# pxl-th/Trace.jl

Measured on AMD Instinct MI355X. Metric: Mray/s (all bounces), higher is better.
Workload: dtype f32

## Files before the change

### trace.jl_amd/csrc/th_device.h

```cpp
#pragma once
#include "th_scene.h"

namespace th {

template <class T>
TH_D T uniform_load(const T* p, uint32_t i) {
#if defined(__HIP_DEVICE_COMPILE__)
    typedef const __attribute__((address_space(4))) T* ConstPtr;
    return ((ConstPtr)(uintptr_t)p)[i];
#else
    return p[i];
#endif
}


struct TriTest {
    float t;
    f3 bary;
};
TH_D bool tri_degenerate(f3 v0, f3 v1, f3 v2) {
    const f3 v = cross(v2 - v0, v1 - v0);
    return dot(v, v) == 0.0f;
}
struct RayShear {
// ... 438 lines not shown
        const float d_o = dot(wo, wh), d_i = dot(wi, wh);
        if (d_o * d_i > 0.0f) return 0.0f;
        const float denom = d_o + eta * d_i;
        const float dwh_dwi = fabs_(d_i * (eta * eta) / (denom * denom));
        return tr_pdf(l.a, l.b, wo, wh) * dwh_dwi;
    }
    default: return same_hemisphere(wo, wi) ? fabs_(cos_theta(wi)) * kInvPi : 0.0f;
    }
}
struct LobeSample {
    f3 wi;
    float pdf;
    f3 f;
    int sampled_type;
};
TH_D LobeSample lobe_sample_f(const Lobe& l, f3 wo, f2 u) {
    LobeSample s;
    s.wi = splat3(0.0f);
    s.pdf = 0.0f;
    s.f = splat3(0.0f);
    s.sampled_type = -1;
    switch (l.kind) {
    case LOBE_SPECULAR_R: {
        s.wi = mk3(-wo.x, -wo.y, wo.z);
        s.pdf = 1.0f;
        s.f = lobe_fresnel(l, cos_theta(s.wi)) * lobe_r(l) / fabs_(cos_theta(s.wi));
        return s;
    }
    case LOBE_SPECULAR_T: {
        const bool entering = cos_theta(wo) > 0.0f;
        const float eta_i = entering ? l.eta_a : l.eta_b;
        const float eta_t = entering ? l.eta_b : l.eta_a;
        f3 wi;
        if (!refract(wo, face_forward(mk3(0.0f, 0.0f, 1.0f), wo), eta_i / eta_t, wi)) return s;
        s.wi = wi;
        s.pdf = 1.0f;
        const float cos_wi = cos_theta(wi);
// ... 244 lines not shown
    if (wo.z == 0.0f) return r;
    f3 wi = cosine_sample_hemisphere(ur);
    if (wo.z < 0.0f) wi = mk3(wi.x, wi.y, -wi.z);
    const float pdf = same_hemisphere(wo, wi) ? fabs_(cos_theta(wi)) * kInvPi : 0.0f;
    if (pdf == 0.0f) return r;
    const f3 wi_w = bsdf_to_world(s, wi);
    const bool refl = (dot(wi_w, s.ng) * dot(wo_w, s.ng)) > 0.0f;
    f3 f = splat3(0.0f);
    if (refl) f = f + lobe_r(l) * kInvPi;
    r.wi = wi_w;
    r.f = f;
    r.pdf = pdf;
    r.sampled_type = l.type;
    return r;
}

struct LightSample {
    f3 radiance;
    f3 wi;
    float pdf;
};
template <bool DIRL>
TH_D LightSample sample_li(const LightRec& l, f3 p) {
    LightSample s;
    const f3 lp = mk3(l.position[0], l.position[1], l.position[2]);
    if (DIRL && l.kind == 2) {
        s.wi = lp;
        s.pdf = 1.0f;
        s.radiance = mk3(l.I[0], l.I[1], l.I[2]);
        return s;
// ... 33 lines not shown
```

### trace.jl_amd/csrc/th_host.h

```cpp
#pragma once
#include <hip/hip_runtime.h>

#include <algorithm>
#include <chrono>
#include <cstdarg>
#include <cstdio>
#include <cstdlib>
#include <cstring>
#include <memory>
#include <string>
#include <thread>
#include <type_traits>
#include <vector>

#include "th_options.h"
#include "th_owned.h"
#include "th_bvh.h"
#include "th_kernels.h"
#include "th_trace2.h"
#include "th_trace8.h"
#ifdef TRHIP_EXPERIMENTS
#include "th_trace4.h"
#include "th_trace7.h"
#endif
// ... 68 lines not shown
struct SceneGeometry {
    uint64_t id = 0;
    int max_node_primitives = -1;
    std::vector<MaterialRec> materials;
    std::vector<float> base_colour;
    std::vector<HostPrim> prims;
    std::vector<float> prim_tan, prim_uv;
    std::vector<SphereRec> spheres;
    std::vector<HostAABB> sphere_bounds;
    FlatBVH bvh;
    FlatBVH acc;
    std::vector<uint32_t> occ_slots;
    std::vector<float> occ_boxes;
    DevBuf d_leaf_boxes;
    DevBuf d_nodes, d_prims, d_nrm, d_tan, d_shade, d_spheres, d_materials, d_base_colour, d_wnodes, d_w8nodes, d_w8tris;
    DevBuf d_acc_w4nodes;
    DevBuf d_acc_wnodes, d_acc_prims, d_slot_boxes, d_sphere_boxes, d_sphere_slots, d_sphere_cert;
};
static_assert(!std::is_copy_constructible_v<SceneGeometry>, "SceneGeometry owns its device buffers");

struct SceneViews {
    bool has_materialless_prim = false;
    DeviceScene dev{};
    WideScene wide{};
    Wide8Scene w8{};
    uint32_t w8_nodes = 0, w8_depth = 0;
    bool partial_spheres = false;
    bool wide_ok = false;
    bool w8_ok = false;
    bool literal_only = false;
// ... 287 lines not shown
```

### trace.jl_amd/csrc/th_kernels.h

```cpp
#pragma once
#include "th_device.h"

namespace th {

constexpr int kBlock = 256;
constexpr int kStackLds = 32;
constexpr int kStackSpill = 32;

struct PathQueue {
    float4* o;
    float4* d;
    float4* beta;
};
struct ShadowQueue {
    float4* o;
    float4* d;
    float4* c;
};
constexpr int kMaxDepth = 62;
constexpr int kSeg = 32;
constexpr uint32_t kSegGran = 256;
#ifndef TH_CTR_STRIDE
#define TH_CTR_STRIDE 32
#endif
// ... 399 lines not shown
            occluded[i] = occ ? 1 : 0;
        }
    }
    if (ctr) {
        if (blockIdx.x == 0 && threadIdx.x == 0) atomicAdd(&ctr->shadow_total, (unsigned long long)seg_total(sv));
        if (COUNT) {
            const unsigned long long sn = wave_sum(nn), spr = wave_sum(np);
            if (lane_id() == 0) {
                atomicAdd(&ctr->nodes_shadow, sn);
                atomicAdd(&ctr->prims_shadow, spr);
            }
        }
    }
}

template <bool TRI_ONLY = false, bool TAN = true>
TH_D bool rebuild_shading(const DeviceScene& sc, int prim, f3 o, f3 d, Shading& sh, uint32_t& material, const float4* bary = nullptr, f3* fast_r = nullptr) {
    const float4* rec = sc.shade + 8 * (size_t)prim;
    const float4 p0 = rec[0], p1 = rec[1], p2 = rec[2];
    const float4 na = rec[3], nb = rec[4], nc = rec[5];
    const float4 cn = rec[6], cs = rec[7];
    const uint32_t meta = __float_as_uint(p0.w);
    material = meta & PRIM_MATERIAL_MASK;
    if (fast_r) *fast_r = mk3(na.w, nb.w, nc.w);
    if (!TRI_ONLY && (meta & PRIM_SPHERE)) {
        const SphereRec& s = sc.spheres[__float_as_uint(p0.x)];
        SphereHit h;
        if (!sphere_intersect<true>(s, o, d, kInf, h)) return false;
        sh = shade_sphere(s, h, d);
        return true;
    }
    const f3 v0 = mk3(p0.x, p0.y, p0.z), v1 = mk3(p1.x, p1.y, p1.z), v2 = mk3(p2.x, p2.y, p2.z);
    TriTest tt;
    if (bary)
        tt.bary = mk3(bary->z, bary->w, bary->x);
    else if (!tri_intersect<true>(v0, v1, v2, o, d, kInf, &tt))
        return false;
    const bool has_n = (meta & PRIM_HAS_NORMALS) != 0;
    const TriConstants tc{mk3(cn.x, cn.y, cn.z), mk3(cs.x, cs.y, cs.z)};
    const float4* tan = (TAN && sc.tri_tan && (meta & PRIM_HAS_TANGENTS)) ? sc.tri_tan + 3 * (size_t)prim : nullptr;
    sh = shade_triangle(v0, v1, v2, has_n, mk3(na.x, na.y, na.z), mk3(nb.x, nb.y, nb.z), mk3(nc.x, nc.y, nc.z), (meta & PRIM_FLIP) != 0, tt.bary, d, &tc, tan);
    return true;
}
template <int TH_ONE_COPY = 0> __global__ __launch_bounds__(kBlock) void k_shade_constants(float4* __restrict__ shade, const float4* __restrict__ prims, const float4* __restrict__ nrm, const float4* __restrict__ uv, uint32_t n_prims) {
    for (uint32_t k = blockIdx.x * kBlock + threadIdx.x; k < n_prims; k += gridDim.x * kBlock) {
        float4* rec = shade + 8 * (size_t)k;
        const float4 p0 = prims[3 * (size_t)k], p1 = prims[3 * (size_t)k + 1], p2 = prims[3 * (size_t)k + 2];
        rec[0] = p0;
        rec[1] = p1;
        rec[2] = p2;
        for (int j = 0; j < 3; ++j) rec[3 + j] = nrm[3 * (size_t)k + j];
        float4 c6 = make_float4(0.0f, 0.0f, 0.0f, 0.0f), c7 = c6;
        if (!(__float_as_uint(p0.w) & PRIM_SPHERE)) {
            float uvs[6];
            bool has_uv = false;
// ... 2 lines not shown
                uvs[0] = a.x, uvs[1] = a.y, uvs[2] = a.z, uvs[3] = a.w, uvs[4] = b.x, uvs[5] = b.y;
                has_uv = b.z != 0.0f;
            }
            const TriConstants tc = triangle_constants(mk3(p0.x, p0.y, p0.z), mk3(p1.x, p1.y, p1.z), mk3(p2.x, p2.y, p2.z), has_uv ? uvs : nullptr);
            c6 = make_float4(tc.n.x, tc.n.y, tc.n.z, 0.0f);
            c7 = make_float4(tc.ss.x, tc.ss.y, tc.ss.z, 0.0f);
        }
        rec[6] = c6;
        rec[7] = c7;
    }
}

#ifndef TH_SHADE_WAVES
#define TH_SHADE_WAVES 4
#endif
struct ShadeStream {
    const uint32_t* tags_in;
    uint32_t* tags_out;
    uint32_t term_stride;
    uint8_t* poison;
};
struct ShadeOut {
    bool want_shadow, want_next;
    float4 so4, sd4, sc4, no4, nd4, nb4;
    uint32_t next_depth;
};
template <bool STREAM, bool FAST, bool TAN = true, bool DIRL = false>
TH_D void shade_vertex(const DeviceScene& sc, const PathQueue& qin, const float4* __restrict__ hits, float4* __restrict__ L, uint32_t i, int depth_fixed, int max_depth,
                       uint32_t hits_have_bary, const ShadeStream& ss, ShadeOut& out) {
    const float4 h4 = hits[i];
    const int prim = __float_as_int(h4.y);
    const float4 o4 = qin.o[i], d4 = qin.d[i], b4 = qin.beta[i];
    const int depth = STREAM ? (int)ss.tags_in[i] : depth_fixed;
    const uint32_t slot = STREAM ? (uint32_t)(depth - 1) * ss.term_stride + __float_as_uint(o4.w) : __float_as_uint(o4.w);
    const f3 o = mk3(o4.x, o4.y, o4.z), d = mk3(d4.x, d4.y, d4.z);
    f3 beta = mk3(b4.x, b4.y, b4.z);
    Shading sh;
    uint32_t material;
    f3 fast_r;
    if (!(rebuild_shading<FAST, TAN>(sc, prim, o, d, sh, material, hits_have_bary ? &h4 : nullptr, &fast_r) && material != PRIM_NO_MATERIAL)) return;
    const LobeSet& bsdf = sc.materials[FAST ? 0u : material].set[1];
    const bool lambert = FAST || bsdf_is_single_lambert(bsdf);
    Lobe lam;
    if (FAST) {
        lam.kind = LOBE_LAMBERT_R;
        lam.type = BSDF_DIFFUSE | BSDF_REFLECTION;
        lam.r[0] = fast_r.x;
        lam.r[1] = fast_r.y;
        lam.r[2] = fast_r.z;
    } else if (lambert) {
        lam = bsdf.lobe[0];
    }
    const uint64_t key = ((uint64_t)__float_as_uint(b4.w) << 32) | (uint64_t)__float_as_uint(d4.w);
    const uint32_t v = (uint32_t)(depth - 1);
    const f3 wo = -d;
    const uint32_t poison = ((isnan_(beta.x) || isinf_(beta.x)) ? 1u : 0u) | ((isnan_(beta.y) || isinf_(beta.y)) ? 2u : 0u) | ((isnan_(beta.z) || isinf_(beta.z)) ? 4u : 0u);
    bool direct_added = false;
    if (sc.n_lights > 0) {
        const int nl = (int)sc.n_lights;
        int ln = (int)__builtin_ceilf(ts_uniform(key, ts_vertex_dim(v, TS_V_LIGHT_PICK)) * (float)nl);
        if (ln > nl) ln = nl;
        if (ln < 1) ln = 1;
        const float light_pdf = 1.0f / (float)nl;
        const LightRec light = nl == 1 ? uniform_load(sc.lights, 0u) : sc.lights[ln - 1];
        const LightSample ls = sample_li<DIRL>(light, sh.p);
        if (ls.pdf > 0.0f && !is_black(ls.radiance)) {
            const f3 f = (lambert ? lambert_bsdf_f(lam, sh, sh.wo, ls.wi) : bsdf_f(bsdf, sh, sh.wo, ls.wi, BSDF_ALL & ~BSDF_SPECULAR)) * fabs_(dot(ls.wi, sh.ns));
            if (!is_black(f)) {
                const f3 fl = f * ls.radiance;
                const f3 Ld1 = splat3(0.0f) + (ls.pdf == 1.0f ? fl : fl / ls.pdf);
                const f3 Ld = light_pdf == 1.0f ? Ld1 : Ld1 / light_pdf;
                const f3 c = beta * Ld;
                const f3 lp = light_target<DIRL>(light, sh.p);
// ... 8 lines not shown
            }
        }
    }
    if (!direct_added && poison && ss.poison) {
        ss.poison[slot] |= (uint8_t)poison;
    } else if (!direct_added && poison) {
        float4 l = L[slot];
        const float nanv = __builtin_nanf("");
        if (poison & 1u) l.x += nanv;
        if (poison & 2u) l.y += nanv;
        if (poison & 4u) l.z += nanv;
        L[slot] = l;
    }
    if (depth < max_depth) {
        const f2 u{ts_uniform(key, ts_vertex_dim(v, TS_V_BSDF_U0)), ts_uniform(key, ts_vertex_dim(v, TS_V_BSDF_U1))};
        const BsdfSample bs = lambert ? lambert_bsdf_sample_f(lam, sh, wo, u) : bsdf_sample_f(bsdf, sh, wo, u, BSDF_ALL);
        if (!(bs.pdf == 0.0f || is_black(bs.f))) {
            beta = beta * (bs.f * fabs_(dot(bs.wi, sh.ns)) / bs.pdf);
            const float by = to_Y(beta);
            bool alive = true;
            if (by < 0.25f) {
                const float cont = jmin(1.0f, by);
                if (ts_uniform(key, ts_vertex_dim(v, TS_V_RR)) > cont)
                    alive = false;
                else
                    beta = beta / cont;
            }
            if (alive) {
                const f3 org = sh.p + 1e-6f * bs.wi;
                const f3 nd = check_direction(bs.wi);
                out.no4 = make_float4(org.x, org.y, org.z, o4.w);
                out.nd4 = make_float4(nd.x, nd.y, nd.z, d4.w);
                out.nb4 = make_float4(beta.x, beta.y, beta.z, b4.w);
                out.next_depth = (uint32_t)(depth + 1);
                out.want_next = true;
            }
        }
    }
}

template <bool STREAM, bool TAN = true, bool DIRL = false>
__global__ __launch_bounds__(kBlock) __attribute__((amdgpu_waves_per_eu(TH_SHADE_WAVES))) void k_shade_path(DeviceScene sc, const DeviceSensor* __restrict__ sep, PathQueue qin, PathQueue qout, ShadowQueue sq, uint32_t cap,
                                                       const float4* __restrict__ hits, float4* __restrict__ L, Counters* ctr, int row, int depth_fixed, int max_depth, uint32_t hits_have_bary,
                                                       ShadeStream ss) {
    __shared__ SegView sv;
    __shared__ uint32_t s_ring[kBlock / 64][128];
    const SegQueue qv{ctr->n_queue[row], cap, 0u};
    seg_load(qv, sv);
    const uint32_t total = sv.prefix[kSeg];
    const uint32_t lane = lane_id(), wv = threadIdx.x >> 6;
    const unsigned long long lt_mask = (1ull << lane) - 1ull;
    const uint32_t seg_out = ((blockIdx.x * kBlock + threadIdx.x) >> 6) % kSeg;
    uint32_t ring_head = 0, ring_cnt = 0;
    auto emit = [&](const ShadeOut& e) {
        uint32_t si, ni;
        wave_compact2(e.want_shadow, &ctr->n_shadow[row][seg_out * kCtrStride], e.want_next, &ctr->n_queue[row + 1][seg_out * kCtrStride], si, ni);
        si += seg_out * cap;
        ni += seg_out * cap;
        if (e.want_shadow) {
            sq.o[si] = e.so4;
            sq.d[si] = e.sd4;
            sq.c[si] = e.sc4;
        }
        if (e.want_next) {
            qout.o[ni] = e.no4;
            qout.d[ni] = e.nd4;
            qout.beta[ni] = e.nb4;
            if (STREAM) ss.tags_out[ni] = e.next_depth;
        }
    };
    uint32_t seg_in = 0;
    for (uint32_t flat = blockIdx.x * kBlock + threadIdx.x; flat < total; flat += gridDim.x * kBlock) {
        uint32_t lb;
        seg_locate_from(sv, flat & ~63u, seg_in, lb);
        const uint32_t local = lb + (flat & 63u);
        const uint32_t i = seg_in * cap + local;
        int cls = 0;
        if (local < sv.count[seg_in]) {
            const int prim = __float_as_int(hits[i].y);
            if (prim >= 0) {
                cls = (__float_as_uint(sc.shade[8 * (size_t)prim].w) & PRIM_FAST) ? 1 : 2;
            }
        }
        ShadeOut e;
        e.want_shadow = e.want_next = false;
        e.next_depth = 0;
        if (cls == 1) shade_vertex<STREAM, true, TAN, DIRL>(sc, qin, hits, L, i, depth_fixed, max_depth, hits_have_bary, ss, e);
        emit(e);
        const unsigned long long m2 = __ballot(cls == 2);
        if (m2) {
            if (cls == 2) s_ring[wv][(ring_head + ring_cnt + (uint32_t)__popcll(m2 & lt_mask)) & 127u] = i;
            ring_cnt += (uint32_t)__popcll(m2);
            __builtin_amdgcn_fence(__ATOMIC_ACQ_REL, "wavefront");
            if (ring_cnt >= 64u) {
                const uint32_t j = s_ring[wv][(ring_head + lane) & 127u];
                ShadeOut g;
                g.want_shadow = g.want_next = false;
                g.next_depth = 0;
                shade_vertex<STREAM, false, TAN, DIRL>(sc, qin, hits, L, j, depth_fixed, max_depth, hits_have_bary, ss, g);
                emit(g);
                ring_head = (ring_head + 64u) & 127u;
                ring_cnt -= 64u;
                __builtin_amdgcn_fence(__ATOMIC_ACQ_REL, "wavefront");
            }
        }
    }
    if (ring_cnt) {
        ShadeOut g;
        g.want_shadow = g.want_next = false;
        g.next_depth = 0;
        if (lane < ring_cnt) shade_vertex<STREAM, false, TAN, DIRL>(sc, qin, hits, L, s_ring[wv][(ring_head + lane) & 127u], depth_fixed, max_depth, hits_have_bary, ss, g);
        emit(g);
    }
}
template <int TH_ONE_COPY = 0> __global__ __launch_bounds__(kBlock) void k_fold_terms(const float4* __restrict__ terms, uint64_t n_slots, uint32_t n_depths, float4* __restrict__ L) {
    for (uint64_t i = (uint64_t)blockIdx.x * kBlock + threadIdx.x; i < n_slots; i += (uint64_t)gridDim.x * kBlock) {
        float4 l = make_float4(0.0f, 0.0f, 0.0f, 0.0f);
        for (uint32_t dd = 0; dd < n_depths; ++dd) {
            const float4 t = terms[(uint64_t)dd * n_slots + i];
            l.x += t.x;
            l.y += t.y;
            l.z += t.z;
        }
        L[i] = l;
    }
}
template <int TH_ONE_COPY = 0> __global__ __launch_bounds__(kBlock) void k_fill_u32(uint32_t* __restrict__ p, uint64_t n, uint32_t v) {
// ... 503 lines not shown
```

### trace.jl_amd/csrc/th_scene.h

```cpp
#pragma once
#include "th_math.h"

namespace th {

enum : uint32_t {
    PRIM_SPHERE = 1u << 24,
    PRIM_HAS_NORMALS = 1u << 25,
    PRIM_FLIP = 1u << 26,
    PRIM_DEGENERATE = 1u << 27,
    PRIM_FAST = 1u << 28,
    PRIM_HAS_TANGENTS = 1u << 29,
    PRIM_MATERIAL_MASK = 0x00ffffffu,
    PRIM_NO_MATERIAL = 0x00ffffffu
};

struct SphereRec {
    float o2w[16];
    float o2w_inv[16];
    float radius, z_min, z_max, theta_min, theta_max, phi_max;
    uint32_t flip;
    uint32_t never_clipped;
};

enum LobeKind : int32_t { LOBE_LAMBERT_R = 0, LOBE_OREN_NAYAR = 1, LOBE_SPECULAR_R = 2, LOBE_SPECULAR_T = 3, LOBE_FRESNEL_SPECULAR = 4, LOBE_MICROFACET_R = 5, LOBE_MICROFACET_T = 6, LOBE_LAMBERT_T = 7 };
enum : int32_t { BSDF_NONE = 0, BSDF_REFLECTION = 1, BSDF_TRANSMISSION = 2, BSDF_DIFFUSE = 4, BSDF_GLOSSY = 8, BSDF_SPECULAR = 16, BSDF_ALL = 31 };
enum : int32_t { FRESNEL_NOOP = 0, FRESNEL_DIELECTRIC = 1 };
// ... 27 lines not shown
};
static_assert(sizeof(LightRec) == 112, "LightRec: the single-light path loads it through scalar loads (th_kernels.h)");

struct DeviceScene {
    const float4* nodes;
    const float4* prims;
    const float4* tri_nrm;
    const float4* tri_tan;
    const float4* shade;
    const SphereRec* spheres;
    const MaterialRec* materials;
    const LightRec* lights;
    uint32_t n_nodes, n_prims, n_spheres, n_materials, n_lights;
};

struct DeviceSensor {
    float raster_to_camera[16];
    float camera_to_world[16];
    float lens_radius, focal_distance, shutter_open, shutter_close;
    float crop_min[2], crop_max[2];
    float filter_radius[2];
    float scale;
    int32_t sb_min[2], sb_max[2];
    int32_t sb_w, sb_h;
    int32_t film_w, film_h;
    int32_t tiles_x, tiles_y;
    int32_t band_y0, band_rows, band_ty0, band_ty1, accumulate;
};

}
// ... 1 lines not shown
```

### trace.jl_amd/csrc/tu_path.hip

```cpp
#include "th_host.h"
#include "th_adaptive.h"

void derive_sensor(const trhip_sensor* sn, DeviceSensor& d) {
    std::memcpy(d.raster_to_camera, sn->raster_to_camera, sizeof d.raster_to_camera);
    std::memcpy(d.camera_to_world, sn->camera_to_world, sizeof d.camera_to_world);
    d.lens_radius = sn->lens_radius;
    d.focal_distance = sn->focal_distance;
    d.shutter_open = sn->shutter_open;
    d.shutter_close = sn->shutter_close;
    for (int i = 0; i < 2; ++i) {
        d.crop_min[i] = sn->crop_min[i];
        d.crop_max[i] = sn->crop_max[i];
        d.filter_radius[i] = sn->filter_radius[i];
        d.sb_min[i] = (int)std::floor(sn->crop_min[i] + 0.5f - sn->filter_radius[i]);
        d.sb_max[i] = (int)std::ceil(sn->crop_max[i] - 0.5f + sn->filter_radius[i]);
    }
    d.scale = sn->scale;
    d.sb_w = d.sb_max[0] - d.sb_min[0] + 1;
    d.sb_h = d.sb_max[1] - d.sb_min[1] + 1;
    d.film_w = (int)std::fabs(sn->crop_max[0] - (sn->crop_min[0] - 1.0f));
    d.film_h = (int)std::fabs(sn->crop_max[1] - (sn->crop_min[1] - 1.0f));
    d.tiles_x = (int)std::floor(((float)(d.sb_max[0] - d.sb_min[0]) + 16.0f) / 16.0f);
    d.tiles_y = (int)std::floor(((float)(d.sb_max[1] - d.sb_min[1]) + 16.0f) / 16.0f);
    d.band_y0 = d.sb_min[1];
    d.band_rows = d.sb_h;
    d.band_ty0 = 0;
    d.band_ty1 = d.tiles_y - 1;
    d.accumulate = 0;
}

bool film_packed(const DeviceSensor& ds) { return std::fmax(ds.filter_radius[0], ds.filter_radius[1]) <= 1.0f && ds.filter_radius[0] > 0.0f && ds.filter_radius[1] > 0.0f; }
static double film_sample_bytes(bool packed) { return packed ? 16.0 : 24.0; }
int ensure_film_samples(trhip_ctx* ctx, bool packed, uint64_t total_slots) { return packed ? 0 : ensure(ctx, ctx->pfilm, total_slots * sizeof(float2)); }
static uint64_t film_padded_slots(const DeviceSensor& ds, uint32_t spp) { return (((uint64_t)ds.sb_w * ds.band_rows + 63u) / 64u) * 64u * spp; }
static bool film_fusable(const DeviceSensor& ds, uint32_t spp) { return film_packed(ds) && film_padded_slots(ds, spp) < (1ull << 32); }
static bool film_fused(const trhip_ctx* ctx, const DeviceSensor& ds, uint32_t spp) { return ctx->opt.film_fused && ctx->opt.film_relayout && film_fusable(ds, spp); }
static FilmSideTable film_side_table(trhip_ctx* ctx, hipStream_t st, uint64_t total_slots, bool* ok) {
    const uint32_t side_cap = (uint32_t)std::min<uint64_t>(total_slots / 16 + 65536, 0x7ffffff0ull);
    *ok = ensure(ctx, ctx->film_side, ((size_t)side_cap + 1) * sizeof(uint4)) == 0;
    if (!*ok) return FilmSideTable{nullptr, nullptr, 0};
    (void)hipMemsetAsync(ctx->film_side.p, 0, sizeof(uint4), st);
    return FilmSideTable{(uint4*)ctx->film_side.p + 1, (uint32_t*)ctx->film_side.p, side_cap};
}
void launch_film(trhip_ctx* ctx, hipStream_t st, const DeviceSensor& ds, const DeviceSensor* dsp, const float4* L, uint64_t total_slots, uint32_t spp, uint64_t seed, uint32_t sample_offset,
                 float4* d_film, bool fused, const MapFrame* map) {
// ... 192 lines not shown
        HIP_TRY(ctx, hipMemcpyAsync(frozen, ctr->n_queue[r], row_bytes, hipMemcpyDeviceToDevice, ps));
        HIP_TRY(ctx, hipMemsetAsync(&lc[out_pg], 0, sizeof(uint32_t), ps));
        HIP_TRY(ctx, hipMemsetAsync(&lc[2], 0, sizeof(uint32_t), ps));
        StreamCtl sc_c{list_of(0, in_pg), list_of(0, out_pg), &lc[in_pg], &lc[2], &lc[out_pg], budget_min, ctx->opt.stream_budget_shift, pq[cur].beta, tags[cur], pq[cur].o, pq[cur].d, pq[cur].beta, hits, tags[cur],
                       ctr->n_queue[r], cap};
        const SegQueue qc{frozen, cap, 0u};
        const TraceOut oc{hits, nullptr, nullptr, nullptr, 1u};
        tm.begin(1, ps);
        launch_trace2_stream(ctx, ps, scene, false, qc, pq[cur].o, pq[cur].d, oc, ctr->work_closest[r], pp.overflow[0].p, ctr, sc_c);
        tm.end(1, ps);
        if (ps2 != ps && r > 0) HIP_TRY(ctx, hipStreamWaitEvent(ps, pp.ev_any, 0));
        tm.begin(2, ps);
        const ShadeStream sst{tags[cur], tags[cur ^ 1], (uint32_t)total_slots};
        if (has_directional_light(scene)) {
            if (scene->dev.tri_tan)
                hipLaunchKernelGGL((k_shade_path<true, true, true>), dim3(g_shade), dim3(kBlock), 0, ps, scene->dev, dsp, pq[cur], pq[cur ^ 1], sq, cap, hits, terms, ctr, r, 0, max_depth, 1u, sst);
            else
                hipLaunchKernelGGL((k_shade_path<true, false, true>), dim3(g_shade), dim3(kBlock), 0, ps, scene->dev, dsp, pq[cur], pq[cur ^ 1], sq, cap, hits, terms, ctr, r, 0, max_depth, 1u, sst);
        } else if (scene->dev.tri_tan) {
            hipLaunchKernelGGL(k_shade_path<true>, dim3(g_shade), dim3(kBlock), 0, ps, scene->dev, dsp, pq[cur], pq[cur ^ 1], sq, cap, hits, terms, ctr, r, 0, max_depth, 1u, sst);
        } else {
            hipLaunchKernelGGL((k_shade_path<true, false>), dim3(g_shade), dim3(kBlock), 0, ps, scene->dev, dsp, pq[cur], pq[cur ^ 1], sq, cap, hits, terms, ctr, r, 0, max_depth, 1u, sst);
        }
        tm.end(2, ps);
        if (ps2 != ps) {
            HIP_TRY(ctx, hipEventRecord(pp.ev_shade, ps));
            HIP_TRY(ctx, hipStreamWaitEvent(ps2, pp.ev_shade, 0));
        }
        HIP_TRY(ctx, hipMemsetAsync(&lc[4 + out_pg], 0, sizeof(uint32_t), ps2));
        HIP_TRY(ctx, hipMemsetAsync(&lc[6], 0, sizeof(uint32_t), ps2));
        StreamCtl sc_a{list_of(1, in_pg), list_of(1, out_pg), &lc[4 + in_pg], &lc[6], &lc[4 + out_pg], budget_min, ctx->opt.stream_budget_shift, nullptr, nullptr, nullptr, nullptr, nullptr, nullptr, nullptr, nullptr, 0u};
        const SegQueue qa{ctr->n_shadow[r], cap, 0u};
        const TraceOut oa{nullptr, terms, sq.c, nullptr, 0u};
        tm.begin(3, ps2);
        launch_trace2_stream(ctx, ps2, scene, true, qa, sq.o, sq.d, oa, ctr->work_shadow[r], pp.overflow[1].p, ctr, sc_a);
        tm.end(3, ps2);
        if (ps2 != ps) HIP_TRY(ctx, hipEventRecord(pp.ev_any, ps2));
// ... 202 lines not shown
            hipLaunchKernelGGL(k_raygen, dim3(grid_for(ctx, nb, 8)), dim3(kBlock), 0, ps, dsp, (uint32_t)j0, (uint32_t)nb, seed, sample_offset, pq[0], cap, ctr, fused ? L : nullptr, spp, fside);
        tm.end(0, ps);
        int cur = 0;
        for (int depth = 1; depth <= max_depth; ++depth) {
            const ShadowQueue& sq = sqs[depth & 1];
            tm.begin(1, ps);
            launch_trace(ctx, ps, scene, false, SegQueue{ctr->n_queue[depth - 1], cap, 0u}, pq[cur].o, pq[cur].d, nullptr,
                         TraceOut{hits, nullptr, nullptr, nullptr, bary_mode, depth == 1 && far_camera(scene, sensor) ? 1u : 0u}, ctr->work_closest[depth - 1], ctr, pp.overflow[0].p);
            tm.end(1, ps);
            if (two && depth > 2) HIP_TRY(ctx, hipStreamWaitEvent(ps, ev_anys[depth & 1], 0));
            tm.begin(2, ps);
            if (envf_in) launch_path_escape(ctx, ps, ctr->n_queue[depth - 1], cap, pq[cur], hits, depth, envf.rec);
            const ShadeStream sst{nullptr, nullptr, 0u, two ? (uint8_t*)ctx->poison.p : nullptr};
            if (has_directional_light(scene)) {
                if (scene->dev.tri_tan)
                    hipLaunchKernelGGL((k_shade_path<false, true, true>), dim3(g_shade), dim3(kBlock), 0, ps, scene->dev, dsp, pq[cur], pq[cur ^ 1], sq, cap, hits, L, ctr, depth - 1, depth, max_depth, bary_mode, sst);
                else
                    hipLaunchKernelGGL((k_shade_path<false, false, true>), dim3(g_shade), dim3(kBlock), 0, ps, scene->dev, dsp, pq[cur], pq[cur ^ 1], sq, cap, hits, L, ctr, depth - 1, depth, max_depth, bary_mode, sst);
            } else if (scene->dev.tri_tan) {
                hipLaunchKernelGGL(k_shade_path<false>, dim3(g_shade), dim3(kBlock), 0, ps, scene->dev, dsp, pq[cur], pq[cur ^ 1], sq, cap, hits, L, ctr, depth - 1, depth, max_depth, bary_mode, sst);
            } else {
                hipLaunchKernelGGL((k_shade_path<false, false>), dim3(g_shade), dim3(kBlock), 0, ps, scene->dev, dsp, pq[cur], pq[cur ^ 1], sq, cap, hits, L, ctr, depth - 1, depth, max_depth, bary_mode, sst);
            }
            tm.end(2, ps);
            if (two) {
                HIP_TRY(ctx, hipEventRecord(pp.ev_shade, ps));
                HIP_TRY(ctx, hipStreamWaitEvent(ps2, pp.ev_shade, 0));
            }
            tm.begin(3, ps2);
            launch_trace(ctx, ps2, scene, true, SegQueue{ctr->n_shadow[depth - 1], cap, 0u}, sq.o, sq.d, nullptr, TraceOut{nullptr, L, sq.c, nullptr}, ctr->work_shadow[depth - 1], ctr, pp.overflow[1].p);
            tm.end(3, ps2);
            if (two) HIP_TRY(ctx, hipEventRecord(ev_anys[depth & 1], ps2));
            cur ^= 1;
        }
        if (two) {
            HIP_TRY(ctx, hipStreamWaitEvent(ps, ev_anys[max_depth & 1], 0));
            if (max_depth >= 2) HIP_TRY(ctx, hipStreamWaitEvent(ps, ev_anys[(max_depth - 1) & 1], 0));
// ... 264 lines not shown
```

### trace.jl_amd/csrc/tu_scene.hip

```cpp
#include "th_host.h"
#include "th_bvh_ref.h"

static uint32_t wide_node_order(const FlatBVH& t, int layout, std::vector<uint32_t>& widx) {
    const uint32_t n = (uint32_t)t.a.size();
    widx.assign(n, 0u);
    auto interior = [&](uint32_t i) { return (t.flags[i] & 3u) != 3u; };
    uint32_t next = 0;
    if (layout != 1) {
        for (uint32_t i = 0; i < n; ++i)
            if (interior(i)) widx[i] = next++;
        return next;
    }
    if (n == 0 || !interior(0)) return 0;
    widx[0] = next++;
    std::vector<uint32_t> stack{0u};
    while (!stack.empty()) {
        const uint32_t i = stack.back();
        stack.pop_back();
        const uint32_t c0 = i + 1, c1 = t.a[i];
        const bool i0 = c0 < n && interior(c0), i1 = c1 < n && interior(c1);
        if (i0 && i1) {
            next = (next + 1u) & ~1u;
            widx[c0] = next++;
            widx[c1] = next++;
// ... 186 lines not shown
float det3(const float* m) {
    return m[0] * (m[5] * m[10] - m[6] * m[9]) - m[1] * (m[4] * m[10] - m[6] * m[8]) + m[2] * (m[4] * m[9] - m[5] * m[8]);
}

bool has_sphere_subtree(const trhip_scene* s, uint32_t root) {
    const uint32_t n_nodes = (uint32_t)s->g->bvh.a.size(), n_prims = (uint32_t)s->g->bvh.order.size();
    if (root >= n_nodes) return true;
    uint32_t end = root;
    while ((s->g->bvh.flags[end] & 3u) != 3u) end = s->g->bvh.a[end];
    for (uint32_t i = root; i <= end && i < n_nodes; ++i)
        if ((s->g->bvh.flags[i] & 3u) == 3u)
            for (uint32_t k = s->g->bvh.a[i]; k < s->g->bvh.a[i] + (s->g->bvh.flags[i] >> 2) && k < n_prims; ++k)
                if (s->g->prims[s->g->bvh.order[k]].kind == 1) return true;
    return false;
}
}

int upload_scene(trhip_scene* s) {
    trhip_ctx* ctx = s->ctx;
    CommitClock clk;
    const uint32_t n_nodes = (uint32_t)s->g->bvh.a.size(), n_prims = (uint32_t)s->g->bvh.order.size();
    RawArray<float4> nodes((size_t)n_nodes * 2), prims((size_t)n_prims * 3), nrm((size_t)n_prims * 3);
    parallel_for(n_nodes, [&](size_t i0, size_t i1) {
        for (size_t i = i0; i < i1; ++i) {
            const float* b = &s->g->bvh.bounds[6 * i];
            nodes[2 * i] = make_float4(b[0], b[1], b[2], __builtin_bit_cast(float, s->g->bvh.a[i]));
            nodes[2 * i + 1] = make_float4(b[3], b[4], b[5], __builtin_bit_cast(float, s->g->bvh.flags[i]));
        }
    });
    parallel_for(n_prims, [&](size_t k0, size_t k1) {
        for (size_t k = k0; k < k1; ++k) {
            const HostPrim& p = s->g->prims[s->g->bvh.order[k]];
            if (p.kind == 1) {
                prims[3 * k] = make_float4(__builtin_bit_cast(float, p.sphere_id), 0, 0, __builtin_bit_cast(float, p.meta));
                prims[3 * k + 1] = prims[3 * k + 2] = make_float4(0, 0, 0, 0);
                nrm[3 * k] = nrm[3 * k + 1] = nrm[3 * k + 2] = make_float4(0, 0, 0, 0);
            } else {
                prims[3 * k] = make_float4(p.v[0], p.v[1], p.v[2], __builtin_bit_cast(float, p.meta));
                prims[3 * k + 1] = make_float4(p.v[3], p.v[4], p.v[5], 0);
                prims[3 * k + 2] = make_float4(p.v[6], p.v[7], p.v[8], 0);
                const uint32_t mat = p.meta & PRIM_MATERIAL_MASK;
                const bool fast = mat != PRIM_NO_MATERIAL && mat < s->g->materials.size() && s->g->materials[mat].set[1].n == 1 && s->g->materials[mat].set[1].lobe[0].kind == LOBE_LAMBERT_R;
                if (fast) prims[3 * k].w = __builtin_bit_cast(float, p.meta | PRIM_FAST);
                for (int j = 0; j < 3; ++j) nrm[3 * k + j] = make_float4(p.n[3 * j], p.n[3 * j + 1], p.n[3 * j + 2], fast ? s->g->materials[mat].set[1].lobe[0].r[j] : 0.0f);
            }
        }
    });
    clk.tick("upload: node / prim records");
    if (int rc = upload(ctx, s->g->d_nodes, nodes.data(), nodes.size() * sizeof(float4))) return rc;
    if (int rc = upload(ctx, s->g->d_prims, prims.data(), prims.size() * sizeof(float4))) return rc;
    if (int rc = upload(ctx, s->g->d_nrm, nrm.data(), nrm.size() * sizeof(float4))) return rc;
    clk.tick("upload: 3 copies");
    const bool any_tan = !s->g->prim_tan.empty(), any_uv = !s->g->prim_uv.empty();
    if (any_tan) s->g->prim_tan.resize(9 * s->g->prims.size(), 0.0f);
    if (any_uv) s->g->prim_uv.resize(7 * s->g->prims.size(), 0.0f);
    s->has_materialless_prim = false;
    for (const HostPrim& p : s->g->prims) s->has_materialless_prim = s->has_materialless_prim || (p.meta & PRIM_MATERIAL_MASK) == PRIM_NO_MATERIAL;
    s->dev.tri_tan = nullptr;
// ... 38 lines not shown
    if (int rc = upload(ctx, s->g->d_spheres, s->g->spheres.data(), s->g->spheres.size() * sizeof(SphereRec))) return rc;
    if (int rc = upload(ctx, s->g->d_materials, s->g->materials.data(), s->g->materials.size() * sizeof(MaterialRec))) return rc;
    if (int rc = upload(ctx, s->g->d_base_colour, s->g->base_colour.data(), s->g->base_colour.size() * sizeof(float))) return rc;
    s->dev.nodes = (const float4*)s->g->d_nodes.p;
    s->dev.prims = (const float4*)s->g->d_prims.p;
    s->dev.tri_nrm = (const float4*)s->g->d_nrm.p;
    s->dev.shade = (const float4*)s->g->d_shade.p;
    s->dev.spheres = (const SphereRec*)s->g->d_spheres.p;
    s->dev.materials = (const MaterialRec*)s->g->d_materials.p;
    s->dev.lights = nullptr;
    s->dev.n_nodes = n_nodes;
    s->dev.n_prims = n_prims;
    s->dev.n_spheres = (uint32_t)s->g->spheres.size();
    s->dev.n_materials = (uint32_t)s->g->materials.size();
    s->dev.n_lights = 0;
    bool has_empty_leaf = false;
    s->wide_ok = false;
    std::memset(&s->wide, 0, sizeof s->wide);
    s->wide.root_ref = kRefNone;
    if (n_nodes > 0 && n_prims < (1u << 24) && !s->literal_only) {
        std::vector<uint32_t> widx;
        const uint32_t n_int = wide_node_order(s->g->bvh, ctx->opt.node_layout, widx);
        bool ok = n_int < (1u << 24);
        RawArray<float4> wn((size_t)n_int * 4);
        if (ctx->opt.node_layout == 1 && ok) std::memset((void*)wn.data(), 0, (size_t)n_int * 4 * sizeof(float4));
        has_empty_leaf = false;
        std::vector<uint8_t> has_sphere(n_nodes, 0);
        if (!s->g->spheres.empty()) {
            std::vector<uint32_t> sphere_slots;
            std::mutex lock;
// ... 1324 lines not shown
```

Measured before the change: 6116.

## Add specialized specular shading path and slim the shade kernel's scene argument

Primitives whose material is a single specular lobe are tagged with a new PRIM_SPEC bit at upload. The shade kernel parks them in the per-wave ring alongside generic hits and tracks how many generic entries are in each batch. A batch containing only specular hits runs a specialized shade_vertex that skips light sampling and the generic BSDF dispatch. The kernel now takes a smaller ShadeScene argument, with the rarely used sphere, material and tangent pointers moved behind a device-side indirection, and the loop bounds are made wave-uniform with readfirstlane. The costs are extra kernel instantiations, more code size and register pressure, an extra dependent load for cold pointers, and more complex ring bookkeeping.

```diff
diff --git a/trace.jl_amd/csrc/th_device.h b/trace.jl_amd/csrc/th_device.h
--- a/trace.jl_amd/csrc/th_device.h
+++ b/trace.jl_amd/csrc/th_device.h
@@ -476,13 +476,14 @@
     f3 f;
     int sampled_type;
 };
+template <int KIND = -1>
 TH_D LobeSample lobe_sample_f(const Lobe& l, f3 wo, f2 u) {
     LobeSample s;
     s.wi = splat3(0.0f);
     s.pdf = 0.0f;
     s.f = splat3(0.0f);
     s.sampled_type = -1;
-    switch (l.kind) {
+    switch (KIND >= 0 ? KIND : l.kind) {
     case LOBE_SPECULAR_R: {
         s.wi = mk3(-wo.x, -wo.y, wo.z);
         s.pdf = 1.0f;
@@ -757,6 +758,26 @@
     r.sampled_type = l.type;
     return r;
 }
+TH_D bool bsdf_has_non_specular(const LobeSet& b) { return bsdf_num_components(b, BSDF_ALL & ~BSDF_SPECULAR) > 0; }
+TH_D BsdfSample specular_bsdf_sample_f(const Lobe& l, const Shading& s, f3 wo_w, f2 u) {
+    BsdfSample r;
+    r.wi = splat3(0.0f);
+    r.f = splat3(0.0f);
+    r.pdf = 0.0f;
+    r.sampled_type = BSDF_NONE;
+    const f2 ur{jmin(u.x * 1.0f - 0.0f, 1.0f), u.y};
+    const f3 wo = bsdf_to_local(s, wo_w);
+    if (wo.z == 0.0f) return r;
+    const LobeSample ls = l.kind == LOBE_SPECULAR_R   ? lobe_sample_f<LOBE_SPECULAR_R>(l, wo, ur)
+                          : l.kind == LOBE_SPECULAR_T ? lobe_sample_f<LOBE_SPECULAR_T>(l, wo, ur)
+                                                      : lobe_sample_f<LOBE_FRESNEL_SPECULAR>(l, wo, ur);
+    if (ls.pdf == 0.0f) return r;
+    r.wi = bsdf_to_world(s, ls.wi);
+    r.f = ls.f;
+    r.pdf = ls.pdf;
+    r.sampled_type = ls.sampled_type >= 0 ? ls.sampled_type : l.type;
+    return r;
+}
 
 struct LightSample {
     f3 radiance;
diff --git a/trace.jl_amd/csrc/th_host.h b/trace.jl_amd/csrc/th_host.h
--- a/trace.jl_amd/csrc/th_host.h
+++ b/trace.jl_amd/csrc/th_host.h
@@ -106,6 +106,7 @@
     std::vector<float> occ_boxes;
     DevBuf d_leaf_boxes;
     DevBuf d_nodes, d_prims, d_nrm, d_tan, d_shade, d_spheres, d_materials, d_base_colour, d_wnodes, d_w8nodes, d_w8tris;
+    DevBuf d_shade_cold;
     DevBuf d_acc_w4nodes;
     DevBuf d_acc_wnodes, d_acc_prims, d_slot_boxes, d_sphere_boxes, d_sphere_slots, d_sphere_cert;
 };
diff --git a/trace.jl_amd/csrc/th_kernels.h b/trace.jl_amd/csrc/th_kernels.h
--- a/trace.jl_amd/csrc/th_kernels.h
+++ b/trace.jl_amd/csrc/th_kernels.h
@@ -437,8 +437,21 @@
     }
 }
 
-template <bool TRI_ONLY = false, bool TAN = true>
-TH_D bool rebuild_shading(const DeviceScene& sc, int prim, f3 o, f3 d, Shading& sh, uint32_t& material, const float4* bary = nullptr, f3* fast_r = nullptr) {
+struct ShadeScene {
+    const float4* shade;
+    const LightRec* lights;
+    uint32_t n_lights;
+    const ShadeCold* cold;
+};
+TH_D const SphereRec* scene_spheres(const DeviceScene& sc) { return sc.spheres; }
+TH_D const MaterialRec* scene_materials(const DeviceScene& sc) { return sc.materials; }
+TH_D const float4* scene_tri_tan(const DeviceScene& sc) { return sc.tri_tan; }
+TH_D const SphereRec* scene_spheres(const ShadeScene& sc) { return sc.cold->spheres; }
+TH_D const MaterialRec* scene_materials(const ShadeScene& sc) { return sc.cold->materials; }
+TH_D const float4* scene_tri_tan(const ShadeScene& sc) { return sc.cold->tri_tan; }
+
+template <bool TRI_ONLY = false, bool TAN = true, class Scene>
+TH_D bool rebuild_shading(const Scene& sc, int prim, f3 o, f3 d, Shading& sh, uint32_t& material, const float4* bary = nullptr, f3* fast_r = nullptr) {
     const float4* rec = sc.shade + 8 * (size_t)prim;
     const float4 p0 = rec[0], p1 = rec[1], p2 = rec[2];
     const float4 na = rec[3], nb = rec[4], nc = rec[5];
@@ -447,7 +460,7 @@
     material = meta & PRIM_MATERIAL_MASK;
     if (fast_r) *fast_r = mk3(na.w, nb.w, nc.w);
     if (!TRI_ONLY && (meta & PRIM_SPHERE)) {
-        const SphereRec& s = sc.spheres[__float_as_uint(p0.x)];
+        const SphereRec& s = scene_spheres(sc)[__float_as_uint(p0.x)];
         SphereHit h;
         if (!sphere_intersect<true>(s, o, d, kInf, h)) return false;
         sh = shade_sphere(s, h, d);
@@ -461,7 +474,8 @@
         return false;
     const bool has_n = (meta & PRIM_HAS_NORMALS) != 0;
     const TriConstants tc{mk3(cn.x, cn.y, cn.z), mk3(cs.x, cs.y, cs.z)};
-    const float4* tan = (TAN && sc.tri_tan && (meta & PRIM_HAS_TANGENTS)) ? sc.tri_tan + 3 * (size_t)prim : nullptr;
+    const float4* tan_base = (TAN && (meta & PRIM_HAS_TANGENTS)) ? scene_tri_tan(sc) : nullptr;
+    const float4* tan = tan_base ? tan_base + 3 * (size_t)prim : nullptr;
     sh = shade_triangle(v0, v1, v2, has_n, mk3(na.x, na.y, na.z), mk3(nb.x, nb.y, nb.z), mk3(nc.x, nc.y, nc.z), (meta & PRIM_FLIP) != 0, tt.bary, d, &tc, tan);
     return true;
 }
@@ -494,6 +508,9 @@
 #ifndef TH_SHADE_WAVES
 #define TH_SHADE_WAVES 4
 #endif
+#ifndef TH_SHADE_SPEC
+#define TH_SHADE_SPEC 1
+#endif
 struct ShadeStream {
     const uint32_t* tags_in;
     uint32_t* tags_out;
@@ -505,9 +522,11 @@
     float4 so4, sd4, sc4, no4, nd4, nb4;
     uint32_t next_depth;
 };
-template <bool STREAM, bool FAST, bool TAN = true, bool DIRL = false>
-TH_D void shade_vertex(const DeviceScene& sc, const PathQueue& qin, const float4* __restrict__ hits, float4* __restrict__ L, uint32_t i, int depth_fixed, int max_depth,
+enum : int { SHADE_GENERIC = 0, SHADE_FAST = 1, SHADE_SPEC = 2 };
+template <bool STREAM, int MODE, bool TAN = true, bool DIRL = false>
+TH_D void shade_vertex(const ShadeScene& sc, const PathQueue& qin, const float4* __restrict__ hits, float4* __restrict__ L, uint32_t i, int depth_fixed, int max_depth,
                        uint32_t hits_have_bary, const ShadeStream& ss, ShadeOut& out) {
+    constexpr bool FAST = MODE == SHADE_FAST, SPEC = MODE == SHADE_SPEC;
     const float4 h4 = hits[i];
     const int prim = __float_as_int(h4.y);
     const float4 o4 = qin.o[i], d4 = qin.d[i], b4 = qin.beta[i];
@@ -519,8 +538,8 @@
     uint32_t material;
     f3 fast_r;
     if (!(rebuild_shading<FAST, TAN>(sc, prim, o, d, sh, material, hits_have_bary ? &h4 : nullptr, &fast_r) && material != PRIM_NO_MATERIAL)) return;
-    const LobeSet& bsdf = sc.materials[FAST ? 0u : material].set[1];
-    const bool lambert = FAST || bsdf_is_single_lambert(bsdf);
+    const LobeSet& bsdf = scene_materials(sc)[FAST ? 0u : material].set[1];
+    const bool lambert = FAST || (!SPEC && bsdf_is_single_lambert(bsdf));
     Lobe lam;
     if (FAST) {
         lam.kind = LOBE_LAMBERT_R;
@@ -528,7 +547,7 @@
         lam.r[0] = fast_r.x;
         lam.r[1] = fast_r.y;
         lam.r[2] = fast_r.z;
-    } else if (lambert) {
+    } else if (SPEC || lambert) {
         lam = bsdf.lobe[0];
     }
     const uint64_t key = ((uint64_t)__float_as_uint(b4.w) << 32) | (uint64_t)__float_as_uint(d4.w);
@@ -536,7 +555,7 @@
     const f3 wo = -d;
     const uint32_t poison = ((isnan_(beta.x) || isinf_(beta.x)) ? 1u : 0u) | ((isnan_(beta.y) || isinf_(beta.y)) ? 2u : 0u) | ((isnan_(beta.z) || isinf_(beta.z)) ? 4u : 0u);
     bool direct_added = false;
-    if (sc.n_lights > 0) {
+    if (!SPEC && sc.n_lights > 0 && (lambert || bsdf_has_non_specular(bsdf))) {
         const int nl = (int)sc.n_lights;
         int ln = (int)__builtin_ceilf(ts_uniform(key, ts_vertex_dim(v, TS_V_LIGHT_PICK)) * (float)nl);
         if (ln > nl) ln = nl;
@@ -575,7 +594,7 @@
     }
     if (depth < max_depth) {
         const f2 u{ts_uniform(key, ts_vertex_dim(v, TS_V_BSDF_U0)), ts_uniform(key, ts_vertex_dim(v, TS_V_BSDF_U1))};
-        const BsdfSample bs = lambert ? lambert_bsdf_sample_f(lam, sh, wo, u) : bsdf_sample_f(bsdf, sh, wo, u, BSDF_ALL);
+        const BsdfSample bs = SPEC ? specular_bsdf_sample_f(lam, sh, wo, u) : lambert ? lambert_bsdf_sample_f(lam, sh, wo, u) : bsdf_sample_f(bsdf, sh, wo, u, BSDF_ALL);
         if (!(bs.pdf == 0.0f || is_black(bs.f))) {
             beta = beta * (bs.f * fabs_(dot(bs.wi, sh.ns)) / bs.pdf);
             const float by = to_Y(beta);
@@ -601,14 +620,14 @@
 }
 
 template <bool STREAM, bool TAN = true, bool DIRL = false>
-__global__ __launch_bounds__(kBlock) __attribute__((amdgpu_waves_per_eu(TH_SHADE_WAVES))) void k_shade_path(DeviceScene sc, const DeviceSensor* __restrict__ sep, PathQueue qin, PathQueue qout, ShadowQueue sq, uint32_t cap,
+__global__ __launch_bounds__(kBlock) __attribute__((amdgpu_waves_per_eu(TH_SHADE_WAVES))) void k_shade_path(ShadeScene sc, const DeviceSensor* __restrict__ sep, PathQueue qin, PathQueue qout, ShadowQueue sq, uint32_t cap,
                                                        const float4* __restrict__ hits, float4* __restrict__ L, Counters* ctr, int row, int depth_fixed, int max_depth, uint32_t hits_have_bary,
                                                        ShadeStream ss) {
     __shared__ SegView sv;
     __shared__ uint32_t s_ring[kBlock / 64][128];
     const SegQueue qv{ctr->n_queue[row], cap, 0u};
     seg_load(qv, sv);
-    const uint32_t total = sv.prefix[kSeg];
+    const uint32_t total = (uint32_t)__builtin_amdgcn_readfirstlane((int)sv.prefix[kSeg]);
     const uint32_t lane = lane_id(), wv = threadIdx.x >> 6;
     const unsigned long long lt_mask = (1ull << lane) - 1ull;
     const uint32_t seg_out = ((blockIdx.x * kBlock + threadIdx.x) >> 6) % kSeg;
@@ -630,48 +649,59 @@
             if (STREAM) ss.tags_out[ni] = e.next_depth;
         }
     };
-    uint32_t seg_in = 0;
-    for (uint32_t flat = blockIdx.x * kBlock + threadIdx.x; flat < total; flat += gridDim.x * kBlock) {
-        uint32_t lb;
-        seg_locate_from(sv, flat & ~63u, seg_in, lb);
-        const uint32_t local = lb + (flat & 63u);
-        const uint32_t i = seg_in * cap + local;
-        int cls = 0;
-        if (local < sv.count[seg_in]) {
-            const int prim = __float_as_int(hits[i].y);
-            if (prim >= 0) {
-                cls = (__float_as_uint(sc.shade[8 * (size_t)prim].w) & PRIM_FAST) ? 1 : 2;
-            }
-        }
-        ShadeOut e;
-        e.want_shadow = e.want_next = false;
-        e.next_depth = 0;
-        if (cls == 1) shade_vertex<STREAM, true, TAN, DIRL>(sc, qin, hits, L, i, depth_fixed, max_depth, hits_have_bary, ss, e);
-        emit(e);
-        const unsigned long long m2 = __ballot(cls == 2);
-        if (m2) {
-            if (cls == 2) s_ring[wv][(ring_head + ring_cnt + (uint32_t)__popcll(m2 & lt_mask)) & 127u] = i;
-            ring_cnt += (uint32_t)__popcll(m2);
-            __builtin_amdgcn_fence(__ATOMIC_ACQ_REL, "wavefront");
-            if (ring_cnt >= 64u) {
-                const uint32_t j = s_ring[wv][(ring_head + lane) & 127u];
-                ShadeOut g;
-                g.want_shadow = g.want_next = false;
-                g.next_depth = 0;
-                shade_vertex<STREAM, false, TAN, DIRL>(sc, qin, hits, L, j, depth_fixed, max_depth, hits_have_bary, ss, g);
-                emit(g);
-                ring_head = (ring_head + 64u) & 127u;
-                ring_cnt -= 64u;
-                __builtin_amdgcn_fence(__ATOMIC_ACQ_REL, "wavefront");
-            }
-        }
-    }
-    if (ring_cnt) {
+    uint32_t ring_gen = 0;
+    auto shade_parked = [&](bool active, bool all_spec) {
+        const uint32_t j = s_ring[wv][(ring_head + lane) & 127u];
         ShadeOut g;
         g.want_shadow = g.want_next = false;
         g.next_depth = 0;
-        if (lane < ring_cnt) shade_vertex<STREAM, false, TAN, DIRL>(sc, qin, hits, L, s_ring[wv][(ring_head + lane) & 127u], depth_fixed, max_depth, hits_have_bary, ss, g);
+        if (TH_SHADE_SPEC && all_spec) {
+            if (active) shade_vertex<STREAM, SHADE_SPEC, TAN, DIRL>(sc, qin, hits, L, j, depth_fixed, max_depth, hits_have_bary, ss, g);
+        } else {
+            if (active) shade_vertex<STREAM, SHADE_GENERIC, TAN, DIRL>(sc, qin, hits, L, j, depth_fixed, max_depth, hits_have_bary, ss, g);
+        }
         emit(g);
+    };
+    uint32_t seg_in = 0;
+    for (uint32_t flat = blockIdx.x * kBlock + threadIdx.x;; flat += gridDim.x * kBlock) {
+        const bool more = (uint32_t)__builtin_amdgcn_readfirstlane((int)flat) < total;
+        uint32_t gen_rest = 0;
+        if (more) {
+            uint32_t lb;
+            seg_locate_from(sv, flat & ~63u, seg_in, lb);
+            const uint32_t local = lb + (flat & 63u);
+            const uint32_t i = seg_in * cap + local;
+            int cls = 0;
+            if (local < sv.count[seg_in]) {
+                const int prim = __float_as_int(hits[i].y);
+                if (prim >= 0) {
+                    const uint32_t meta = __float_as_uint(sc.shade[8 * (size_t)prim].w);
+                    cls = (meta & PRIM_FAST) ? 1 : (TH_SHADE_SPEC && (meta & PRIM_SPEC)) ? 3 : 2;
+                }
+            }
+            ShadeOut e;
+            e.want_shadow = e.want_next = false;
+            e.next_depth = 0;
+            if (cls == 1) shade_vertex<STREAM, SHADE_FAST, TAN, DIRL>(sc, qin, hits, L, i, depth_fixed, max_depth, hits_have_bary, ss, e);
+            emit(e);
+            const unsigned long long m2 = __ballot(cls >= 2);
+            if (m2) {
+                const uint32_t rank = (uint32_t)__popcll(m2 & lt_mask), room = 64u - ring_cnt;
+                if (cls >= 2) s_ring[wv][(ring_head + ring_cnt + rank) & 127u] = i;
+                ring_gen += (uint32_t)__popcll(__ballot(cls == 2 && rank < room));
+                gen_rest = (uint32_t)__popcll(__ballot(cls == 2 && rank >= room));
+                ring_cnt += (uint32_t)__popcll(m2);
+                __builtin_amdgcn_fence(__ATOMIC_ACQ_REL, "wavefront");
+            }
+        }
+        if (ring_cnt >= 64u || (!more && ring_cnt)) {
+            shade_parked(lane < ring_cnt, ring_gen == 0u);
+            ring_head = (ring_head + 64u) & 127u;
+            ring_cnt -= ring_cnt < 64u ? ring_cnt : 64u;
+            ring_gen = gen_rest;
+            __builtin_amdgcn_fence(__ATOMIC_ACQ_REL, "wavefront");
+        }
+        if (!more) break;
     }
 }
 template <int TH_ONE_COPY = 0> __global__ __launch_bounds__(kBlock) void k_fold_terms(const float4* __restrict__ terms, uint64_t n_slots, uint32_t n_depths, float4* __restrict__ L) {
diff --git a/trace.jl_amd/csrc/th_scene.h b/trace.jl_amd/csrc/th_scene.h
--- a/trace.jl_amd/csrc/th_scene.h
+++ b/trace.jl_amd/csrc/th_scene.h
@@ -10,6 +10,7 @@
     PRIM_DEGENERATE = 1u << 27,
     PRIM_FAST = 1u << 28,
     PRIM_HAS_TANGENTS = 1u << 29,
+    PRIM_SPEC = 1u << 30,
     PRIM_MATERIAL_MASK = 0x00ffffffu,
     PRIM_NO_MATERIAL = 0x00ffffffu
 };
@@ -67,6 +68,12 @@
     uint32_t n_nodes, n_prims, n_spheres, n_materials, n_lights;
 };
 
+struct ShadeCold {
+    const SphereRec* spheres;
+    const MaterialRec* materials;
+    const float4* tri_tan;
+};
+
 struct DeviceSensor {
     float raster_to_camera[16];
     float camera_to_world[16];
diff --git a/trace.jl_amd/csrc/tu_path.hip b/trace.jl_amd/csrc/tu_path.hip
--- a/trace.jl_amd/csrc/tu_path.hip
+++ b/trace.jl_amd/csrc/tu_path.hip
@@ -29,6 +29,7 @@
     d.accumulate = 0;
 }
 
+static ShadeScene shade_scene(const trhip_scene* s) { return ShadeScene{s->dev.shade, s->dev.lights, s->dev.n_lights, (const ShadeCold*)s->g->d_shade_cold.p}; }
 bool film_packed(const DeviceSensor& ds) { return std::fmax(ds.filter_radius[0], ds.filter_radius[1]) <= 1.0f && ds.filter_radius[0] > 0.0f && ds.filter_radius[1] > 0.0f; }
 static double film_sample_bytes(bool packed) { return packed ? 16.0 : 24.0; }
 int ensure_film_samples(trhip_ctx* ctx, bool packed, uint64_t total_slots) { return packed ? 0 : ensure(ctx, ctx->pfilm, total_slots * sizeof(float2)); }
@@ -251,13 +252,13 @@
         const ShadeStream sst{tags[cur], tags[cur ^ 1], (uint32_t)total_slots};
         if (has_directional_light(scene)) {
             if (scene->dev.tri_tan)
-                hipLaunchKernelGGL((k_shade_path<true, true, true>), dim3(g_shade), dim3(kBlock), 0, ps, scene->dev, dsp, pq[cur], pq[cur ^ 1], sq, cap, hits, terms, ctr, r, 0, max_depth, 1u, sst);
+                hipLaunchKernelGGL((k_shade_path<true, true, true>), dim3(g_shade), dim3(kBlock), 0, ps, shade_scene(scene), dsp, pq[cur], pq[cur ^ 1], sq, cap, hits, terms, ctr, r, 0, max_depth, 1u, sst);
             else
-                hipLaunchKernelGGL((k_shade_path<true, false, true>), dim3(g_shade), dim3(kBlock), 0, ps, scene->dev, dsp, pq[cur], pq[cur ^ 1], sq, cap, hits, terms, ctr, r, 0, max_depth, 1u, sst);
+                hipLaunchKernelGGL((k_shade_path<true, false, true>), dim3(g_shade), dim3(kBlock), 0, ps, shade_scene(scene), dsp, pq[cur], pq[cur ^ 1], sq, cap, hits, terms, ctr, r, 0, max_depth, 1u, sst);
         } else if (scene->dev.tri_tan) {
-            hipLaunchKernelGGL(k_shade_path<true>, dim3(g_shade), dim3(kBlock), 0, ps, scene->dev, dsp, pq[cur], pq[cur ^ 1], sq, cap, hits, terms, ctr, r, 0, max_depth, 1u, sst);
+            hipLaunchKernelGGL(k_shade_path<true>, dim3(g_shade), dim3(kBlock), 0, ps, shade_scene(scene), dsp, pq[cur], pq[cur ^ 1], sq, cap, hits, terms, ctr, r, 0, max_depth, 1u, sst);
         } else {
-            hipLaunchKernelGGL((k_shade_path<true, false>), dim3(g_shade), dim3(kBlock), 0, ps, scene->dev, dsp, pq[cur], pq[cur ^ 1], sq, cap, hits, terms, ctr, r, 0, max_depth, 1u, sst);
+            hipLaunchKernelGGL((k_shade_path<true, false>), dim3(g_shade), dim3(kBlock), 0, ps, shade_scene(scene), dsp, pq[cur], pq[cur ^ 1], sq, cap, hits, terms, ctr, r, 0, max_depth, 1u, sst);
         }
         tm.end(2, ps);
         if (ps2 != ps) {
@@ -490,13 +491,13 @@
             const ShadeStream sst{nullptr, nullptr, 0u, two ? (uint8_t*)ctx->poison.p : nullptr};
             if (has_directional_light(scene)) {
                 if (scene->dev.tri_tan)
-                    hipLaunchKernelGGL((k_shade_path<false, true, true>), dim3(g_shade), dim3(kBlock), 0, ps, scene->dev, dsp, pq[cur], pq[cur ^ 1], sq, cap, hits, L, ctr, depth - 1, depth, max_depth, bary_mode, sst);
+                    hipLaunchKernelGGL((k_shade_path<false, true, true>), dim3(g_shade), dim3(kBlock), 0, ps, shade_scene(scene), dsp, pq[cur], pq[cur ^ 1], sq, cap, hits, L, ctr, depth - 1, depth, max_depth, bary_mode, sst);
                 else
-                    hipLaunchKernelGGL((k_shade_path<false, false, true>), dim3(g_shade), dim3(kBlock), 0, ps, scene->dev, dsp, pq[cur], pq[cur ^ 1], sq, cap, hits, L, ctr, depth - 1, depth, max_depth, bary_mode, sst);
+                    hipLaunchKernelGGL((k_shade_path<false, false, true>), dim3(g_shade), dim3(kBlock), 0, ps, shade_scene(scene), dsp, pq[cur], pq[cur ^ 1], sq, cap, hits, L, ctr, depth - 1, depth, max_depth, bary_mode, sst);
             } else if (scene->dev.tri_tan) {
-                hipLaunchKernelGGL(k_shade_path<false>, dim3(g_shade), dim3(kBlock), 0, ps, scene->dev, dsp, pq[cur], pq[cur ^ 1], sq, cap, hits, L, ctr, depth - 1, depth, max_depth, bary_mode, sst);
+                hipLaunchKernelGGL(k_shade_path<false>, dim3(g_shade), dim3(kBlock), 0, ps, shade_scene(scene), dsp, pq[cur], pq[cur ^ 1], sq, cap, hits, L, ctr, depth - 1, depth, max_depth, bary_mode, sst);
             } else {
-                hipLaunchKernelGGL((k_shade_path<false, false>), dim3(g_shade), dim3(kBlock), 0, ps, scene->dev, dsp, pq[cur], pq[cur ^ 1], sq, cap, hits, L, ctr, depth - 1, depth, max_depth, bary_mode, sst);
+                hipLaunchKernelGGL((k_shade_path<false, false>), dim3(g_shade), dim3(kBlock), 0, ps, shade_scene(scene), dsp, pq[cur], pq[cur ^ 1], sq, cap, hits, L, ctr, depth - 1, depth, max_depth, bary_mode, sst);
             }
             tm.end(2, ps);
             if (two) {
diff --git a/trace.jl_amd/csrc/tu_scene.hip b/trace.jl_amd/csrc/tu_scene.hip
--- a/trace.jl_amd/csrc/tu_scene.hip
+++ b/trace.jl_amd/csrc/tu_scene.hip
@@ -224,6 +224,11 @@
                 if (s->g->prims[s->g->bvh.order[k]].kind == 1) return true;
     return false;
 }
+bool single_specular(const trhip_scene* s, uint32_t mat) {
+    if (mat == PRIM_NO_MATERIAL || mat >= s->g->materials.size()) return false;
+    const LobeSet& b = s->g->materials[mat].set[1];
+    return b.n == 1 && (b.lobe[0].kind == LOBE_SPECULAR_R || b.lobe[0].kind == LOBE_SPECULAR_T || b.lobe[0].kind == LOBE_FRESNEL_SPECULAR);
+}
 }
 
 int upload_scene(trhip_scene* s) {
@@ -242,7 +247,7 @@
         for (size_t k = k0; k < k1; ++k) {
             const HostPrim& p = s->g->prims[s->g->bvh.order[k]];
             if (p.kind == 1) {
-                prims[3 * k] = make_float4(__builtin_bit_cast(float, p.sphere_id), 0, 0, __builtin_bit_cast(float, p.meta));
+                prims[3 * k] = make_float4(__builtin_bit_cast(float, p.sphere_id), 0, 0, __builtin_bit_cast(float, p.meta | (single_specular(s, p.meta & PRIM_MATERIAL_MASK) ? PRIM_SPEC : 0u)));
                 prims[3 * k + 1] = prims[3 * k + 2] = make_float4(0, 0, 0, 0);
                 nrm[3 * k] = nrm[3 * k + 1] = nrm[3 * k + 2] = make_float4(0, 0, 0, 0);
             } else {
@@ -252,6 +257,7 @@
                 const uint32_t mat = p.meta & PRIM_MATERIAL_MASK;
                 const bool fast = mat != PRIM_NO_MATERIAL && mat < s->g->materials.size() && s->g->materials[mat].set[1].n == 1 && s->g->materials[mat].set[1].lobe[0].kind == LOBE_LAMBERT_R;
                 if (fast) prims[3 * k].w = __builtin_bit_cast(float, p.meta | PRIM_FAST);
+                if (single_specular(s, mat)) prims[3 * k].w = __builtin_bit_cast(float, p.meta | PRIM_SPEC);
                 for (int j = 0; j < 3; ++j) nrm[3 * k + j] = make_float4(p.n[3 * j], p.n[3 * j + 1], p.n[3 * j + 2], fast ? s->g->materials[mat].set[1].lobe[0].r[j] : 0.0f);
             }
         }
@@ -320,6 +326,10 @@
     s->dev.n_spheres = (uint32_t)s->g->spheres.size();
     s->dev.n_materials = (uint32_t)s->g->materials.size();
     s->dev.n_lights = 0;
+    {
+        const ShadeCold cold{s->dev.spheres, s->dev.materials, s->dev.tri_tan};
+        if (int rc = upload(ctx, s->g->d_shade_cold, &cold, sizeof cold)) return rc;
+    }
     bool has_empty_leaf = false;
     s->wide_ok = false;
     std::memset(&s->wide, 0, sizeof s->wide);
```

Result: faster. 6281, median of 6 (+2.7%).
